# IST-DASLab/qutlass

Hardware: AMD Instinct MI355X
Metric: TFLOP/s & %FP4-MFMA-peak, MXFP4 GEMM 4096x4096x4096, 1 MI355X (higher is better)
Workload: dtype fp4 (e2m1 x e2m1, e8m0 block scales, fp32 accumulate, bf16 out); 1 GPU; matmul_mxf4_bf16_tn 4096x4096x4096, gs=32 e8m0 scales (BASELINE.json configs[1]); parallelism=single GPU, clock_ramp=8000 untimed steps (~250 ms) before the 5 warmup steps

## Files before the change

### qutlass_amd/csrc/capi.hip

```cpp
#include <hip/hip_runtime.h>

#include <algorithm>
#include <atomic>
#include <chrono>
#include <cmath>
#include <cstdarg>
#include <cstdio>
#include <cstring>
#include <utility>

#include "../../include/qutlass_amd.h"
#include "gemm_mx.hip.h"
#include "gemm_mx_forms.hip.h"
#include "gemm_mx_deepp.hip.h"
#include "gemm_mx_deepp16.hip.h"
#if QAMD_BENCH
#include "lab/gemm_mx_duo.hip.h"
#include "lab/gemm_mx_deepp_lab.hip.h"
#endif
#include "gemm_mx_skinny.hip.h"
#include "gemm_mx_ks.hip.h"
#include "gemm_mx_os.hip.h"
#include "gemm_mx_os_w4a8.hip.h"
#include "gemm_mx_fusedq.hip.h"
// ... 90 lines not shown
#else
constexpr bool opt_hw_fp4() { return true; }
constexpr int opt_gemm_variant() { return 0; }
constexpr int opt_nvf4_variant() { return 0; }
constexpr int opt_splitk_wg() { return 0; }
constexpr int opt_splitk_min_kt() { return 32; }
constexpr int opt_transpose_nc() { return 0; }
constexpr int opt_pp_shift() { return 2; }
constexpr int opt_pp_flags() { return 1; }
constexpr int opt_quant_wg_per_cu() { return 0; }
constexpr int opt_splitk_force() { return 0; }
constexpr int opt_deepp_grid() { return 0; }
constexpr int opt_bwd_variant() { return 0; }
constexpr int opt_moe_sort_one_launch_max() { return 0; }
constexpr uint32_t* opt_dbg() { return nullptr; }
#endif

inline int64_t cdiv(int64_t a, int64_t b) { return (a + b - 1) / b; }

#if QAMD_DEF(1)
int chip_cus() {
  static std::atomic<int> cache[64];
  int dev = 0;
  if (hipGetDevice(&dev) != hipSuccess || dev < 0 || dev >= 64) return 256;
  int v = cache[dev].load(std::memory_order_relaxed);
  if (v <= 0) {
    int n = 0;
    if (hipDeviceGetAttribute(&n, hipDeviceAttributeMultiprocessorCount, dev) != hipSuccess || n <= 0) n = 256;
    cache[dev].store(n, std::memory_order_relaxed);
    v = n;
  }
  return v;
}
#else
int chip_cus();
#endif


template <class C, int PP>
int launch_gemm(GemmParams p, hipStream_t s) {
  p.tiles_m = (int)cdiv(p.M, C::BM);
  p.tiles_n = (int)cdiv(p.N, C::BN);
  p.raster_magic = raster_magic(p.tiles_n);
  if (PP != 7 && PP != 9) { p.ws = nullptr; p.splits = 1; p.ctr = nullptr; p.tag = 0; }
  hipLaunchKernelGGL((gemm_mx_kernel<C, PP>), dim3(p.tiles_m * p.tiles_n, p.splits), dim3(C::THREADS), 0, s, p);
  return check_launch("gemm_mx_kernel");
}

inline int deepp_grid(int tiles) {
  const int forced = opt_deepp_grid();
  if (forced > 0) return std::min(forced, tiles);
  const int cus = chip_cus();
  const int rounds = (tiles + cus - 1) / cus;
  const int g = ((tiles + rounds - 1) / rounds + 7) / 8 * 8;
  return std::min(std::min(g, cus), tiles);
}

template <class C, bool TRACE = false, int ST_AUX = 0, int LAB = 0, int ONEFORM = 0>
int launch_gemm_deepp(GemmParams p, hipStream_t s) {
  p.tiles_m = (int)cdiv(p.M, C::BM);
  p.tiles_n = (int)cdiv(p.N, C::BN);
  p.raster_magic = raster_magic(p.tiles_n);
  p.ws = nullptr; p.splits = 1; p.ctr = nullptr; p.tag = 0;
  const int grid = deepp_grid(p.tiles_m * p.tiles_n);
#if QAMD_BENCH
#ifdef QAMD_ROUTE_LABK
  if constexpr (!TRACE && LAB == 0) {
    hipLaunchKernelGGL((labk::gemm_mx_deepp_kernel<C, false, ST_AUX, 8>), dim3(grid), dim3(C::THREADS), 0, s, p);
    return check_launch("labk::gemm_mx_deepp_kernel");
  }
#endif
  if constexpr (TRACE || LAB != 0) {
    hipLaunchKernelGGL((labk::gemm_mx_deepp_kernel<C, TRACE, ST_AUX, LAB>), dim3(grid), dim3(C::THREADS), 0, s, p);
    return check_launch("labk::gemm_mx_deepp_kernel");
  }
#else
  static_assert(!TRACE && LAB == 0, "traces / ablations: lab build only");
#endif
  const int64_t kt = cdiv((int64_t)p.K * C::EBITS / 8, 128);
  const bool odd = (kt & 1) && kt >= 3, one = grid == p.tiles_m * p.tiles_n;
  if (odd && one) hipLaunchKernelGGL((gemm_mx_deepp_kernel<C, ST_AUX, true, true>), dim3(grid), dim3(C::THREADS), 0, s, p);
  else if (odd) hipLaunchKernelGGL((gemm_mx_deepp_kernel<C, ST_AUX, true, false>), dim3(grid), dim3(C::THREADS), 0, s, p);
  else if (one) {
    static_assert(ONEFORM == 0 || ONEFORM == 16 || ONEFORM == 32, "one-tile form");
    static_assert(ONEFORM == 0 || QAMD_BENCH, "forced one-tile forms: lab build only");
    if constexpr (ONEFORM == 16 || (ONEFORM == 0 && kDeeppOneTile16)) hipLaunchKernelGGL((gemm_mx_deepp16_kernel<C, ST_AUX>), dim3(grid), dim3(C::THREADS), 0, s, p);
    else hipLaunchKernelGGL((gemm_mx_deepp_kernel<C, ST_AUX, false, true>), dim3(grid), dim3(C::THREADS), 0, s, p);
  }
  else hipLaunchKernelGGL((gemm_mx_deepp_kernel<C, ST_AUX>), dim3(grid), dim3(C::THREADS), 0, s, p);
  return check_launch("gemm_mx_deepp_kernel");
}

#if QAMD_BENCH
template <class C, int ST_AUX = 17, int RET = 0, bool TRACE = false>
int launch_gemm_duo(GemmParams p, hipStream_t s) {
  p.tiles_m = (int)cdiv(p.M, C::BM);
  p.tiles_n = (int)cdiv(p.N, C::BN);
  p.raster_magic = raster_magic(p.tiles_n);
  p.ws = nullptr; p.splits = 1; p.ctr = nullptr; p.tag = 0;
  const int grid = deepp_grid(p.tiles_m * p.tiles_n);
  hipLaunchKernelGGL((gemm_mx_duo_kernel<C, ST_AUX, RET, TRACE>), dim3(grid), dim3(C::THREADS), 0, s, p);
  return check_launch("gemm_mx_duo_kernel");
}
#endif

template <int TM, int TN, int D = 8>
int launch_gemm_ks(GemmParams p, hipStream_t s) {
  using C = KsCfg<TM, TN, D>;
  p.tiles_m = (int)cdiv(p.M, TM);
  p.tiles_n = (int)cdiv(p.N, TN);
  p.ws = nullptr; p.splits = 1; p.ctr = nullptr; p.tag = 0;
  hipLaunchKernelGGL((gemm_mx_ks_kernel<C>), dim3(p.tiles_m * p.tiles_n), dim3(256), 0, s, p);
  return check_launch("gemm_mx_ks_kernel");
}

template <bool RM, int TN, int EBITS, int TM, int AFMT, bool GRP, class P>
void launch_os_by_stages(int64_t KT, dim3 grid, const P& p, hipStream_t s) {
  const dim3 block(256);
  constexpr int SMAX = TM == 32 ? 4 : 3;
  if (KT <= 4) hipLaunchKernelGGL((gemm_mx_os_kernel<OsCfg<1, TN, EBITS, TM, AFMT>, RM, false, GRP>), grid, block, 0, s, p);
  else if (KT <= 8) hipLaunchKernelGGL((gemm_mx_os_kernel<OsCfg<2, TN, EBITS, TM, AFMT>, RM, false, GRP>), grid, block, 0, s, p);
  else if (KT <= 12) hipLaunchKernelGGL((gemm_mx_os_kernel<OsCfg<3, TN, EBITS, TM, AFMT>, RM, false, GRP>), grid, block, 0, s, p);
  else if (KT <= 4 * SMAX) hipLaunchKernelGGL((gemm_mx_os_kernel<OsCfg<SMAX, TN, EBITS, TM, AFMT>, RM, false, GRP>), grid, block, 0, s, p);
  else hipLaunchKernelGGL((gemm_mx_os_kernel<OsCfg<SMAX, TN, EBITS, TM, AFMT>, RM, true, GRP>), grid, block, 0, s, p);
}
template <bool RM = false, int TN = 32, int EBITS = 4, int TM = 32, int AFMT = 0>
int launch_gemm_os(GemmParams p, hipStream_t s) {
  p.tiles_m = (int)cdiv(p.M, TM);
  p.tiles_n = (int)cdiv(p.N, TN);
  p.ws = nullptr; p.splits = 1; p.ctr = nullptr; p.tag = 0;
  launch_os_by_stages<RM, TN, EBITS, TM, AFMT, false>(cdiv((int64_t)p.K * EBITS / 8, 128), dim3(p.tiles_m * p.tiles_n), p, s);
  return check_launch("gemm_mx_os_kernel");
}
template <int EBITS = 4, int AFMT = 0, bool RM = false, int TN = 16>
int launch_gemm_os16(GemmParams p, hipStream_t s) {
  p.tiles_m = (int)cdiv(p.M, 16);
  p.tiles_n = (int)cdiv(p.N, TN);
  p.ws = nullptr; p.splits = 1; p.ctr = nullptr; p.tag = 0;
  const int64_t KT = cdiv((int64_t)p.K * EBITS / 8, 128);
  const dim3 grid(p.tiles_m * p.tiles_n), block(256);
  constexpr int STAGE = Os16Cfg<1, EBITS, AFMT, TN>::STAGE;
  constexpr int SFIT = 160 * 1024 / (4 * STAGE), SMAX = SFIT >= 8 ? 8 : SFIT >= 4 ? 4 : SFIT;
  static_assert(SMAX >= 3, "LDS budget");
  if (KT <= 4) hipLaunchKernelGGL((gemm_mx_os16_kernel<Os16Cfg<1, EBITS, AFMT, TN>, false, RM>), grid, block, 0, s, p);
  else if (KT <= 8) hipLaunchKernelGGL((gemm_mx_os16_kernel<Os16Cfg<2, EBITS, AFMT, TN>, false, RM>), grid, block, 0, s, p);
  else if (KT <= 16 && SMAX >= 4) hipLaunchKernelGGL((gemm_mx_os16_kernel<Os16Cfg<(SMAX >= 4 ? 4 : SMAX), EBITS, AFMT, TN>, false, RM>), grid, block, 0, s, p);
  else if (KT <= 4 * SMAX) hipLaunchKernelGGL((gemm_mx_os16_kernel<Os16Cfg<SMAX, EBITS, AFMT, TN>, false, RM>), grid, block, 0, s, p);
  else hipLaunchKernelGGL((gemm_mx_os16_kernel<Os16Cfg<SMAX, EBITS, AFMT, TN>, true, RM>), grid, block, 0, s, p);
  return check_launch("gemm_mx_os16_kernel");
}
inline const MxFormRow* os16_form(int64_t N, int64_t cus) {
  for (const MxFormRow& f : MX_FORMS)
    if (f.family == MXF_DECODE && cdiv(N, f.tn) <= cus) return &f;
  return nullptr;
}
inline int os16_wide_plan(int ebits, int64_t N, int64_t K, int64_t cus) {
  const MxFormRow* f = os16_form(N, cus);
  const int tn = f ? f->tn : 0;
  const int64_t KT = cdiv(K * ebits / 8, 128);
  if (ebits == 4) {
    if (tn == 32) return (KT >= 12 && KT <= 32) ? f->variant : 0;
    if (tn == 48) return (KT >= 8 && KT <= 24) ? f->variant : 0;
    if (tn == 56) return (KT >= 8 && KT <= 16) ? f->variant : 0;
    if (tn == 64) return (KT >= 8 && KT <= 16) ? f->variant : 0;
    return 0;
  }
  if (tn == 32) return (KT >= 16 && KT <= 64) ? f->variant : 0;
  if (tn == 48) return (KT >= 16 && KT <= 32) ? f->variant : 0;
  return 0;
// ... 255 lines not shown
    return launch_gemm_os<RM, F.tn, EBITS, F.tm, AFMT>(p, s);
  } else {
    static_assert(F.family == MXF_DECODE && Os16Cfg<1, EBITS, AFMT, F.tn>::TM == F.tm && Os16Cfg<1, EBITS, AFMT, F.tn>::TN == F.tn, "the decode configuration is the row's");
    return launch_gemm_os16<EBITS, AFMT, RM, F.tn>(p, s);
  }
}
template <int I, int EBITS, int AFMT, bool RM>
inline bool try_mx_row(int v, const GemmParams& p, hipStream_t s, int& rc) {
  if constexpr (MX_FORMS[I].product && (MX_FORMS[I].ops & mx_op(EBITS, AFMT, RM)) != 0) {
    if (v == MX_FORMS[I].variant) { rc = launch_mx_row<I, EBITS, AFMT, RM>(p, s); return true; }
  }
  return false;
}
template <int EBITS, int AFMT, bool RM, int... I>
int launch_mx_form(int v, const GemmParams& p, hipStream_t s, const char* name, std::integer_sequence<int, I...>) {
  int rc = 0;
  if ((try_mx_row<I, EBITS, AFMT, RM>(v, p, s, rc) || ...)) return rc;
  if (AFMT == 1) return fail(QAMD_ERR_INVALID, "%s: gemm_variant %d has no e5m2-operand instantiation", name, v);
  return fail(QAMD_ERR_INVALID, "%s: unknown gemm_variant %d", name, v);
}

#if QAMD_BENCH
template <int EBITS>
int dispatch_lab_variant(int v, const GemmParams& p, hipStream_t s, const char* name) {
  constexpr bool SPLIT = EBITS == 8;
  switch (v) {
    case 273: return launch_gemm<GemmCfg<128, 128, 2, 2, EBITS, SPLIT, 128, 3>, 9>(p, s);
    case 272: return launch_gemm<GemmCfg<64, 128, 2, 2, EBITS, SPLIT, 128, 3>, 9>(p, s);
    case 270: return launch_gemm<GemmCfg<64, 64, 2, 2, EBITS, SPLIT, 128, 3>, 9>(p, s);
    case 224 + 1000: return launch_gemm<GemmCfg<128, 128, 2, 2, EBITS, SPLIT, 128, 2>, 9>(p, s);
    case 373: return launch_gemm<GemmCfg<128, 128, 2, 4, EBITS, SPLIT, 0, 3>, 9>(p, s);
    case 374: return launch_gemm<GemmCfg<128, 128, 4, 2, EBITS, SPLIT, 0, 3>, 9>(p, s);
    case 325: return launch_gemm<GemmCfg<256, 128, 2, 2, EBITS, SPLIT, 0, 3>, 9>(p, s);
    case 326: return launch_gemm<GemmCfg<128, 256, 2, 2, EBITS, SPLIT, 0, 3>, 9>(p, s);
    case 327: return launch_gemm<GemmCfg<256, 128, 2, 2, EBITS, SPLIT, 0, 2>, 9>(p, s);
    case 76: return launch_gemm<GemmCfg<128, 128, 2, 2, EBITS, SPLIT, 0, 4>, 9>(p, s);
    case 79: return launch_gemm<GemmCfg<64, 128, 2, 2, EBITS, SPLIT, 0, 4>, 9>(p, s);
    case 224: return launch_gemm<GemmCfg<128, 128, 2, 2, EBITS, SPLIT>, 3>(p, s);
    case 225: return launch_gemm<GemmCfg<256, 128, 4, 2, EBITS, SPLIT>, 3>(p, s);
    case 227: return launch_gemm<GemmCfg<128, 64, 2, 2, EBITS, SPLIT>, 3>(p, s);
    case 228: return launch_gemm<GemmCfg<64, 128, 2, 2, EBITS, SPLIT>, 3>(p, s);
    case 229: return launch_gemm<GemmCfg<64, 64, 2, 2, EBITS, SPLIT>, 3>(p, s);
    case 170: return launch_gemm<GemmCfg<64, 64, 2, 2, EBITS, SPLIT, 0, 3>, 7>(p, s);
    case 171: return launch_gemm<GemmCfg<128, 64, 2, 2, EBITS, SPLIT, 0, 3>, 7>(p, s);
    case 172: return launch_gemm<GemmCfg<64, 128, 2, 2, EBITS, SPLIT, 0, 3>, 7>(p, s);
    case 173: return launch_gemm<GemmCfg<128, 128, 2, 2, EBITS, SPLIT, 0, 3>, 7>(p, s);
    case 1: return launch_gemm<GemmCfg<256, 256, 2, 4, EBITS, SPLIT>, 1>(p, s);
    case 2: return launch_gemm<GemmCfg<128, 128, 2, 2, EBITS, SPLIT>, 0>(p, s);
    case 3: return launch_gemm<GemmCfg<256, 128, 4, 2, EBITS, SPLIT>, 0>(p, s);
    case 4: return launch_gemm<GemmCfg<128, 256, 2, 4, EBITS, SPLIT>, 0>(p, s);
    case 5: return launch_gemm<GemmCfg<256, 256, 2, 4, EBITS, SPLIT>, 0>(p, s);
    case 20: return launch_gemm<GemmCfg<256, 256, 2, 4, EBITS, SPLIT>, 3>(p, s);
    case 26: return launch_gemm<GemmCfg<128, 256, 2, 4, EBITS, SPLIT>, 3>(p, s);
    case 74: return launch_gemm<GemmCfg<64, 64, 2, 2, EBITS, SPLIT, 0, 4>, 7>(p, s);
    case 75: return launch_gemm<GemmCfg<64, 64, 2, 2, EBITS, SPLIT, 0, 6>, 7>(p, s);
    case 80: return launch_gemm<GemmCfg<64, 64, 2, 2, EBITS, SPLIT, 1, 3>, 7>(p, s);
    case 81: return launch_gemm<GemmCfg<64, 64, 2, 2, EBITS, SPLIT, 2, 3>, 7>(p, s);
    case 82: return launch_gemm<GemmCfg<64, 64, 2, 2, EBITS, SPLIT, 32, 3>, 7>(p, s);
    case 83: return launch_gemm<GemmCfg<64, 64, 2, 2, EBITS, SPLIT, 34, 3>, 7>(p, s);
    case 84: return launch_gemm<GemmCfg<64, 64, 2, 2, EBITS, SPLIT, 35, 3>, 7>(p, s);
    case 78: return launch_gemm<GemmCfg<64, 64, 2, 2, EBITS, SPLIT, 16, 3>, 7>(p, s);
  }
  if constexpr (EBITS == 8) {
    if (v == 89) return launch_gemm_deepp_sk<GemmCfg<256, 256, 2, 2, 8, true>>(p, s);
    if (v == 30) return launch_gemm<GemmCfg<256, 256, 2, 2, 8, true>, 4>(p, s);
  }
  if constexpr (EBITS == 4) {
    if (v == 89) return launch_gemm_deepp_sk<GemmCfg<256, 256, 2, 2, 4, false>>(p, s);
    if (v == 99) return launch_gemm_hetero<GemmCfg<256, 256, 2, 2, 4, false>, GemmCfg<128, 128, 2, 2, 4, false, 0, 3>, 17>(p, s);
    if (v == 563 || v == 564) {
      const bool deep = cdiv(p.K, 256) > 24;
      if (v == 563) return deep ? launch_gemm_ks<64, 32, 6>(p, s) : launch_gemm_ks<64, 32, 4>(p, s);
      return deep ? launch_gemm_ks<64, 64, 6>(p, s) : launch_gemm_ks<64, 64, 4>(p, s);
    }
    if (v == 565) return launch_gemm_ks<32, 32, 4>(p, s);
    if (v == 566) return launch_gemm_ks<32, 32, 8>(p, s);
    if (v == 567) return launch_gemm_ks<32, 32, 6>(p, s);
    if (v == 88) return launch_gemm_duo<GemmCfg<256, 256, 2, 4, 4, false>, 17, 0>(p, s);
    if (v == 87) return launch_gemm_duo<GemmCfg<256, 256, 2, 4, 4, false>, 17, 1>(p, s);
    if (v == 86) return launch_gemm_duo<GemmCfg<256, 256, 2, 4, 4, false>, 17, 0, true>(p, s);
    if (v == 298) return launch_gemm_hetero<GemmCfg<256, 256, 2, 2, 4, false>, GemmCfg<128, 128, 2, 2, 4, false, 128, 4>, 17>(p, s);
    if (v == 190) return launch_gemm_deepp<GemmCfg<256, 256, 2, 2, 4, false>, false, 17, 0, 32>(p, s);
    if (v == 191) return launch_gemm_deepp<GemmCfg<256, 256, 2, 2, 4, false>, false, 17, 0, 16>(p, s);
    if (v == 91) return launch_gemm_deepp<GemmCfg<256, 256, 2, 2, 4, false>, true, 17>(p, s);
    if (v == 92) return launch_gemm_deepp<GemmCfg<256, 256, 2, 2, 4, false>, false, 2>(p, s);
    if (v == 93) return launch_gemm_deepp<GemmCfg<256, 256, 2, 2, 4, false>, false, 16>(p, s);
    if (v == 94) return launch_gemm_deepp<GemmCfg<256, 256, 2, 2, 4, false>, false, 0>(p, s);
    if (v == 95) return launch_gemm_deepp<GemmCfg<256, 256, 2, 2, 4, false>, false, 19>(p, s);
    if (v == 96) return launch_gemm_deepp<GemmCfg<256, 256, 2, 2, 4, false>, false, 1>(p, s);
    if (v == 97) return launch_gemm_deepp<GemmCfg<256, 256, 2, 2, 4, false>, false, 17, 1>(p, s);
    if (v == 197) return launch_gemm_deepp<GemmCfg<256, 256, 2, 2, 4, false>, false, 17, 2>(p, s);
    if (v == 297) return launch_gemm_deepp<GemmCfg<256, 256, 2, 2, 4, false>, false, 17, 3>(p, s);
    if (v == 397) return launch_gemm_deepp<GemmCfg<256, 256, 2, 2, 4, false>, false, 17, 4>(p, s);
    switch (v) {
      case 6: return launch_gemm<GemmCfg<256, 256, 2, 4, 4, false>, 2>(p, s);
      case 7: return launch_gemm<GemmCfg<128, 128, 2, 2, 4, false>, 2>(p, s);
      case 8: return launch_gemm<GemmCfg<256, 128, 4, 2, 4, false>, 2>(p, s);
      case 9: return launch_gemm<GemmCfg<128, 256, 2, 4, 4, false>, 2>(p, s);
      case 30: return launch_gemm<GemmCfg<256, 256, 2, 2, 4, false>, 4>(p, s);
      case 31: return launch_gemm<GemmCfg<256, 256, 2, 2, 4, false, 8>, 4>(p, s);
      case 32: return launch_gemm<GemmCfg<256, 256, 2, 2, 4, false, 9>, 4>(p, s);
      case 33: return launch_gemm<GemmCfg<256, 256, 2, 2, 4, false, 10>, 4>(p, s);
      case 34: return launch_gemm<GemmCfg<256, 256, 2, 2, 4, false, 40>, 4>(p, s);
      case 40: return launch_gemm<GemmCfg<256, 256, 2, 2, 4, false>, 5>(p, s);
      case 41: return launch_gemm<GemmCfg<256, 256, 2, 2, 4, false, 8>, 5>(p, s);
      case 42: return launch_gemm<GemmCfg<256, 256, 2, 2, 4, false, 9>, 5>(p, s);
      case 43: return launch_gemm<GemmCfg<256, 256, 2, 2, 4, false, 10>, 5>(p, s);
      case 50: return launch_gemm<GemmCfg<256, 256, 2, 4, 4, false, 64>, 3>(p, s);
      case 51: return launch_gemm<GemmCfg<256, 256, 2, 2, 4, false, 64>, 4>(p, s);
      case 52: return launch_gemm<GemmCfg<256, 256, 2, 2, 4, false, 64>, 5>(p, s);
      case 53: return launch_gemm<GemmCfg<256, 256, 2, 2, 4, false, 72>, 5>(p, s);
      case 54: return launch_gemm<GemmCfg<256, 256, 2, 2, 4, false, 73>, 5>(p, s);
      case 55: return launch_gemm<GemmCfg<256, 256, 2, 2, 4, false, 74>, 5>(p, s);
      case 56: return launch_gemm<GemmCfg<256, 256, 2, 2, 4, false, 104>, 5>(p, s);
      case 35: return launch_gemm<GemmCfg<256, 256, 2, 2, 4, false, 16>, 4>(p, s);
      case 36: return launch_gemm<GemmCfg<256, 256, 2, 2, 4, false, 17>, 4>(p, s);
      case 21: return launch_gemm<GemmCfg<256, 256, 2, 4, 4, false, 8>, 3>(p, s);
      case 22: return launch_gemm<GemmCfg<256, 256, 2, 4, 4, false, 9>, 3>(p, s);
      case 23: return launch_gemm<GemmCfg<256, 256, 2, 4, 4, false, 10>, 3>(p, s);
    }
  }
  if constexpr (EBITS == 4 && !SPLIT) {
    const int rc = dispatch_ablation_mx4(v, p, s);
    if (rc >= 0) return rc;
  }
  return fail(QAMD_ERR_INVALID, "%s: unknown gemm_variant %d", name, v);
}
#endif

template <int EBITS, int AFMT, bool RM>
int dispatch_variant(int v, const GemmParams& p, hipStream_t s, const char* name) {
#if QAMD_BENCH
  if constexpr (AFMT == 0 && !RM) {
    if (p.pp_flags & 4096) {
      const MxFormRow* f = mx_form(v);
      if (f && f->family == MXF_RING) v += 100;
      else if (f && f->family == MXF_PIPELINED && f->depth == 2) v += 200;
    }
    if (!mx_form(v)) return dispatch_lab_variant<EBITS>(v, p, s, name);
  }
#endif
  return launch_mx_form<EBITS, AFMT, RM>(v, p, s, name, std::make_integer_sequence<int, MX_NFORMS>());
}

int launch_nn_fused_a5(const GemmParams& p, hipStream_t s, bool per_tile)
#if QAMD_DEF(4)
{
#if QAMD_BENCH
  if (per_tile) return launch_gemm<GemmCfg<256, 256, 2, 2, 8, true, 0, 2, 1>, 6>(p, s);
#endif
  (void)per_tile;
  return launch_gemm_deepp8<GemmCfg<256, 256, 2, 2, 8, true, 0, 2, 1>, true>(p, s);
}
#else
;
#endif

#if QAMD_TU != 0
#if QAMD_TU == 2
template int dispatch_variant<4, 0, false>(int, const GemmParams&, hipStream_t, const char*);
#else
extern template int dispatch_variant<4, 0, false>(int, const GemmParams&, hipStream_t, const char*);
#endif
#if QAMD_TU == 3
template int dispatch_variant<8, 0, false>(int, const GemmParams&, hipStream_t, const char*);
#if QAMD_BENCH
// ... 1638 lines not shown
```

### qutlass_amd/csrc/gemm_mx_deepp16.hip.h

```cpp
#pragma once
#include "gemm_mx_deepp.hip.h"

namespace qamd {

constexpr bool kDeeppOneTile16 = true;

constexpr int deepp16_row_done_at(int s) { return (s >= 7 && s <= 63 && (s - 7) % 8 == 0) ? (s - 7) / 8 : -1; }

template <class C, int ST_AUX = 0>
__device__ __forceinline__ void gemm_mx_deepp16(char* smem, const GemmParams& p, const int bid, const int G, const int ntiles) {
  static_assert(C::EBITS == 4 && C::BM == 256 && C::BN == 256 && C::WAVES_M == 2 && C::WAVES_N == 2 && C::NSTAGE == 2 && C::PPW == 2,
                "persistent deep schedule: fp4, 256x256 tiles, 4 waves of 128x128");
  constexpr int MT = 8, NT = 8;
  constexpr int STAGE = C::STAGE_BYTES, OFF_SCR = DeepPCfg<C>::OFF_SCR;
  GemmCtx<C> cx(smem, p);
  const int lane = cx.lane, wave = cx.wave, r16 = lane & 15, kq = lane >> 4;
  const int KT = cx.KT, KTe = (KT + 1) & ~1, CB = cx.CB, rowbytes = cx.rowbytes;
  const int tile = xcd_remap(bid, G);

  auto fence = [&]() __attribute__((always_inline)) { __builtin_amdgcn_sched_barrier(0); };
  struct Desc { __amdgpu_buffer_rsrc_t a, b, s; };
  int m0, n0;
  {
    int tm, tn;
    raster_decode(tile < ntiles ? tile : ntiles - 1, p.tiles_m, p.tiles_n, p.raster_magic, tm, tn);
    m0 = uniform(tm * C::BM);
    n0 = uniform(tn * C::BN);
  }
  Desc cur;
  {
    const bool valid = tile < ntiles;
    const uint32_t a_off = (uint32_t)m0 * rowbytes, b_off = (uint32_t)n0 * rowbytes;
    const uint32_t sa_off = (uint32_t)(m0 >> 7) * CB * 512, sb_off = (uint32_t)(n0 >> 7) * CB * 512;
    cur.a = make_rsrc(p.A + a_off, valid ? p.a_bytes - a_off : 0u);
    cur.b = make_rsrc(p.B + b_off, valid ? p.b_bytes - b_off : 0u);
    cur.s = cx.sIsB ? make_rsrc(p.SFB + sb_off, valid ? p.sfb_bytes - sb_off : 0u) : make_rsrc(p.SFA + sa_off, valid ? p.sfa_bytes - sa_off : 0u);
  }

  v4f acc[MT][NT];
  v4i fa[2][MT], fb[2][NT];
  v4i xq[2][4];
  const int sh = 8 * kq;

  const int sw = (r16 >> 1) & 7;
  int rdF[2];
#pragma unroll
  for (int h = 0; h < 2; ++h) rdF[h] = (cx.wave_m * C::WTM + r16) * C::ROWB + (((4 * h + kq) ^ sw) << 4);
  const int rdBd = cx.rdBd;
  const int rdSA = C::OFF_S + (cx.wave_m * C::SCT) * 512 + r16 * 16, rdSB = C::OFF_S + (C::PA + cx.wave_n * C::SCT) * 512 + r16 * 16;
  static_assert(C::SCT == 2 && C::WTM == 128 && C::WTN == 128, "a wave's rows are one 128-row scale tile; a stage is two column tiles");

  typedef __attribute__((address_space(3))) const v4i* lds_v4i_t;
  uint32_t rbA = 0, rbB = 0;
  auto read_base = [&](const int buf, const int h) __attribute__((always_inline)) {
    rbA = (uint32_t)(uintptr_t)(lds_ptr_t)(smem + buf * STAGE + rdF[h]);
    rbB = rbA + (uint32_t)rdBd;
    asm volatile("" : "+v"(rbA), "+v"(rbB));
  };
  auto read_frag = [&](const int h, const int i) __attribute__((always_inline)) {
    if (i < MT) fa[h][i] = *(lds_v4i_t)(uintptr_t)(rbA + (uint32_t)(i * 16 * C::ROWB));
    else fb[h][i - MT] = *(lds_v4i_t)(uintptr_t)(rbB + (uint32_t)((i - MT) * 16 * C::ROWB));
  };
  auto read_raw = [&](const int buf, const int h, const int k) __attribute__((always_inline)) {
    xq[h][k] = *(const v4i*)(smem + buf * STAGE + (k < 2 ? rdSA : rdSB) + h * 512 + (k & 1) * 256);
  };
  auto shift1 = [&](const int h, const int k) __attribute__((always_inline)) {
    xq[h][k >> 2][k & 3] = (int)((unsigned)xq[h][k >> 2][k & 3] >> sh);
  };
  auto mfma1 = [&](const int h, const int m, const int n, const bool zero_c) __attribute__((always_inline)) {
    const v4i a = fa[h][m], b = fb[h][n];
    const int sb1 = xq[h][2 + (n & 1)][n >> 1], sa1 = xq[h][m & 1][m >> 1];
    if (zero_c)
      asm volatile("v_mfma_scale_f32_16x16x128_f8f6f4 %0, %1, %2, 0, %3, %4 op_sel_hi:[0,0,0] cbsz:4 blgp:4" : "=a"(acc[m][n]) : "v"(b), "v"(a), "v"(sb1), "v"(sa1));
    else
      asm volatile("v_mfma_scale_f32_16x16x128_f8f6f4 %0, %1, %2, %0, %3, %4 op_sel_hi:[0,0,0] cbsz:4 blgp:4" : "+a"(acc[m][n]) : "v"(b), "v"(a), "v"(sb1), "v"(sa1));
  };

  int vb0 = 0, vb1 = 0, vbS = 0;
  auto dma_prep = [&](int kt, bool valid) __attribute__((always_inline)) {
    int lastmask = (kt == KT - 1) ? -1 : 0;
    int oobm = (valid && kt < KT) ? 0 : -1;
    int oobs = (valid && kt * C::SCT + cx.colS < CB) ? 0 : -1;
    asm volatile("" : "+v"(lastmask), "+v"(oobm), "+v"(oobs));
    vb0 = (((cx.voffT[0] & lastmask) | (cx.voffAB[0] & ~lastmask)) & ~oobm) | ((int)0x80000000 & oobm);
    vb1 = (((cx.voffT[1] & lastmask) | (cx.voffAB[1] & ~lastmask)) & ~oobm) | ((int)0x80000000 & oobm);
    vbS = (cx.voffS & ~oobs) | ((int)0x80000000 & oobs);
  };
  auto dma_item = [&](const Desc& d, int kt, const int buf, const int item) __attribute__((always_inline)) {
    char* st = smem + buf * STAGE;
    if (item < 16) {
      const int t = item & 7, q = wave * 8 + t;
      const int v = ((t & 1) ? vb1 : vb0) + q * cx.rstep;
      __builtin_amdgcn_raw_ptr_buffer_load_lds(item < 8 ? d.a : d.b, (lds_ptr_t)(st + (item < 8 ? 0 : C::OFF_B) + q * 1024), 16, v, kt * C::ROWB, 0, QAMD_DMA_AUX);
    } else {
      __builtin_amdgcn_raw_ptr_buffer_load_lds(d.s, (lds_ptr_t)(st + C::OFF_S + wave * 1024), 16, vbS, kt * C::SCT * 512, 0, 0);
    }
  };
  auto dma_stage = [&](const Desc& d, int kt, bool valid, const int buf) __attribute__((always_inline)) {
    dma_prep(kt, valid);
#pragma unroll
    for (int i = 0; i < 17; ++i) dma_item(d, kt, buf, i);
  };

  auto half = [&](const int h, const bool zero_c, auto extra) __attribute__((always_inline)) {
    int i = 0;
#pragma unroll
    for (int m = 0; m < MT; ++m)
#pragma unroll
      for (int n = 0; n < NT; ++n) {
        mfma1(h, m, n, zero_c);
        extra(i);
        fence();
        ++i;
      }
  };
  auto fill = [&](const int buf, const int hs, const int i) __attribute__((always_inline)) {
    if (i < 32 && (i & 1)) read_frag(hs, i >> 1);
    if (i >= 33 && i < 40 && (i & 1)) read_raw(buf, hs, (i - 33) >> 1);
    if (i >= 46 && i < 62) shift1(hs, i - 46);
  };

  auto stage = [&](auto bufc, auto firstc, int ktl, bool dvalid, auto dmac) __attribute__((always_inline)) {
    constexpr int BUF = decltype(bufc)::value;
    constexpr bool FIRST = decltype(firstc)::value;
    constexpr bool DMA = decltype(dmac)::value;
    read_base(BUF, 1);
    half(0, FIRST, [&](const int i) __attribute__((always_inline)) {
      fill(BUF, 1, i);
      if (DMA && i == 42) dma_prep(ktl, dvalid);
      if (i == 63) read_base(BUF ^ 1, 0);
    });
    asm volatile("s_waitcnt vmcnt(0) lgkmcnt(0)" ::: "memory");
    __builtin_amdgcn_s_barrier();
    fence();
    half(1, false, [&](const int i) __attribute__((always_inline)) {
      fill(BUF ^ 1, 0, i);
      if (DMA && !(i & 1) && i < 34) dma_item(cur, ktl, BUF, i >> 1);
    });
  };

  char* scr = smem + OFF_SCR + wave * DeepPCfg<C>::SCR_PER_WAVE;
  const int scrW = r16 * 512 + ((kq ^ (r16 & 7)) << 4);
  const int rrl = lane >> 3, ccl = lane & 7;
  const int scrR = rrl * 512 + (ccl >> 2) * 128 + ((((2 * ccl) & 7) ^ rrl) << 4);
  const float alpha = *p.alpha;
  __amdgpu_buffer_rsrc_t rD;
  int stLane, colLim;
  {
    const int64_t left = ((int64_t)(p.M - m0) * p.ldd - n0) * 2;
    rD = make_rsrc(p.D + ((int64_t)m0 * p.ldd + n0), (uint32_t)(left > 0x7fffffffll ? 0x7fffffffll : left));
    stLane = ((cx.wave_m * C::WTM + rrl) * p.ldd + cx.wave_n * C::WTN + 8 * ccl) * 2;
    colLim = p.N - n0 - cx.wave_n * C::WTN - 8 * ccl;
  }
  auto retire_write = [&](const int m) __attribute__((always_inline)) {
    asm volatile("s_nop 15" ::: "memory");
#pragma unroll
    for (int n = 0; n < NT; ++n) *(v4f*)(scr + (scrW ^ ((n & 1) << 6)) + (n >> 1) * 128) = acc[m][n];
  };
  v4f rb[2][2];
  auto retire_read = [&](const int rh) __attribute__((always_inline)) {
#pragma unroll
    for (int ch = 0; ch < 2; ++ch) {
      rb[ch][0] = *(const v4f*)(scr + scrR + rh * 4096 + ch * 256);
      rb[ch][1] = *(const v4f*)(scr + (scrR ^ 16) + rh * 4096 + ch * 256);
    }
  };
  auto retire_store = [&](const int m, const int pass) __attribute__((always_inline)) {
    const int rh = pass >> 1, ch = pass & 1;
    const v4f lo = rb[ch][0], hi = rb[ch][1];
    v4i o;
    o[0] = (int)pack_bf16x2(lo[0] * alpha, lo[1] * alpha);
    o[1] = (int)pack_bf16x2(lo[2] * alpha, lo[3] * alpha);
    o[2] = (int)pack_bf16x2(hi[0] * alpha, hi[1] * alpha);
    o[3] = (int)pack_bf16x2(hi[2] * alpha, hi[3] * alpha);
    int ldd2 = p.ldd * 2;
    asm volatile("" : "+s"(ldd2));
    __builtin_amdgcn_raw_buffer_store_b128(__builtin_bit_cast(v4u, o), rD, (64 * ch < colLim) ? stLane : (int)0x80000000, (16 * m + 8 * rh) * ldd2 + 128 * ch, ST_AUX);
  };

  auto final_stage = [&]() __attribute__((always_inline)) {
    read_base(1, 1);
    half(0, false, [&](const int i) __attribute__((always_inline)) { fill(1, 1, i); });
    asm volatile("s_waitcnt vmcnt(0) lgkmcnt(0)" ::: "memory");
    __builtin_amdgcn_s_barrier();
    fence();
    static_for<0, 75>([&](auto sc) __attribute__((always_inline)) {
      constexpr int s = decltype(sc)::value;
      if constexpr (s < 64) mfma1(1, s / 8, s % 8, false);
      constexpr int d1 = s - 1, d3 = s - 3, d5 = s - 5, d6 = s - 6, d7 = s - 7, d9 = s - 9, d10 = s - 10;
      if constexpr (deepp16_row_done_at(d5) >= 0) retire_store(deepp16_row_done_at(d5), 0);
      if constexpr (deepp16_row_done_at(d6) >= 0) retire_store(deepp16_row_done_at(d6), 1);
      if constexpr (deepp16_row_done_at(d9) >= 0) retire_store(deepp16_row_done_at(d9), 2);
      if constexpr (deepp16_row_done_at(d10) >= 0) retire_store(deepp16_row_done_at(d10), 3);
      if constexpr (deepp16_row_done_at(d1) >= 0) retire_write(deepp16_row_done_at(d1));
      if constexpr (deepp16_row_done_at(d3) >= 0) retire_read(0);
      if constexpr (deepp16_row_done_at(d7) >= 0) retire_read(1);
      fence();
    });
  };

  using I0 = std::integral_constant<int, 0>;
  using I1 = std::integral_constant<int, 1>;
  using BT = std::integral_constant<bool, true>;
  using BF = std::integral_constant<bool, false>;

  dma_stage(cur, 0, true, 0);
  dma_stage(cur, 1, true, 1);
  asm volatile("s_waitcnt vmcnt(17)" ::: "memory");
  __builtin_amdgcn_s_barrier();
  fence();
#pragma unroll
  for (int k = 0; k < 4; ++k) read_raw(0, 0, k);
  read_base(0, 0);
#pragma unroll
  for (int i = 0; i < MT + NT; ++i) read_frag(0, i);
#pragma unroll
  for (int k = 0; k < 16; ++k) shift1(0, k);
  fence();

  stage(I0{}, BT{}, 2, true, BT{});
  int kt = 1;
  for (; kt + 4 < KTe; kt += 2) {
    stage(I1{}, BF{}, kt + 2, true, BT{});
    stage(I0{}, BF{}, kt + 3, true, BT{});
  }
  if (kt + 2 < KTe) {
    stage(I1{}, BF{}, kt + 2, true, BT{});
    stage(I0{}, BF{}, 0, false, BF{});
  }
  final_stage();
  asm volatile("s_waitcnt vmcnt(0)" ::: "memory");
}

template <class C, int ST_AUX = 0>
__global__ __launch_bounds__(C::THREADS) void gemm_mx_deepp16_kernel(const GemmParams p) {
  __shared__ __attribute__((aligned(16))) char smem[DeepPCfg<C>::LDS_BYTES];
  asm volatile("" :: "s"(p.A), "s"(p.D), "s"(p.K), "s"(p.b_bytes), "s"((int)gridDim.x));
  gemm_mx_deepp16<C, ST_AUX>(smem, p, (int)blockIdx.x, (int)gridDim.x, p.tiles_m * p.tiles_n);
}

}
```

Baseline: 4357 TFLOP/s.

## Fuse LDS-DMA issue into MFMA asm and spread loads in deepp16 K-loop

Result: faster. 4491 TFLOP/s, median of 6 (+3.1%).

```diff
diff --git a/qutlass_amd/csrc/capi.hip b/qutlass_amd/csrc/capi.hip
--- a/qutlass_amd/csrc/capi.hip
+++ b/qutlass_amd/csrc/capi.hip
@@ -196,9 +196,10 @@
   if (odd && one) hipLaunchKernelGGL((gemm_mx_deepp_kernel<C, ST_AUX, true, true>), dim3(grid), dim3(C::THREADS), 0, s, p);
   else if (odd) hipLaunchKernelGGL((gemm_mx_deepp_kernel<C, ST_AUX, true, false>), dim3(grid), dim3(C::THREADS), 0, s, p);
   else if (one) {
-    static_assert(ONEFORM == 0 || ONEFORM == 16 || ONEFORM == 32, "one-tile form");
+    static_assert(ONEFORM == 0 || ONEFORM == 16 || ONEFORM == 32 || (ONEFORM >= 160 && ONEFORM < 168), "one-tile form");
     static_assert(ONEFORM == 0 || QAMD_BENCH, "forced one-tile forms: lab build only");
-    if constexpr (ONEFORM == 16 || (ONEFORM == 0 && kDeeppOneTile16)) hipLaunchKernelGGL((gemm_mx_deepp16_kernel<C, ST_AUX>), dim3(grid), dim3(C::THREADS), 0, s, p);
+    if constexpr (ONEFORM >= 160) hipLaunchKernelGGL((gemm_mx_deepp16_kernel<C, ST_AUX, ONEFORM - 160>), dim3(grid), dim3(C::THREADS), 0, s, p);
+    else if constexpr (ONEFORM == 16 || (ONEFORM == 0 && kDeeppOneTile16)) hipLaunchKernelGGL((gemm_mx_deepp16_kernel<C, ST_AUX>), dim3(grid), dim3(C::THREADS), 0, s, p);
     else hipLaunchKernelGGL((gemm_mx_deepp_kernel<C, ST_AUX, false, true>), dim3(grid), dim3(C::THREADS), 0, s, p);
   }
   else hipLaunchKernelGGL((gemm_mx_deepp_kernel<C, ST_AUX>), dim3(grid), dim3(C::THREADS), 0, s, p);
@@ -620,6 +621,12 @@
     if (v == 298) return launch_gemm_hetero<GemmCfg<256, 256, 2, 2, 4, false>, GemmCfg<128, 128, 2, 2, 4, false, 128, 4>, 17>(p, s);
     if (v == 190) return launch_gemm_deepp<GemmCfg<256, 256, 2, 2, 4, false>, false, 17, 0, 32>(p, s);
     if (v == 191) return launch_gemm_deepp<GemmCfg<256, 256, 2, 2, 4, false>, false, 17, 0, 16>(p, s);
+    if (v == 192) return launch_gemm_deepp<GemmCfg<256, 256, 2, 2, 4, false>, false, 17, 0, 160>(p, s);
+    if (v == 193) return launch_gemm_deepp<GemmCfg<256, 256, 2, 2, 4, false>, false, 17, 0, 160 + KL_SCALES>(p, s);
+    if (v == 194) return launch_gemm_deepp<GemmCfg<256, 256, 2, 2, 4, false>, false, 17, 0, 160 + KL_DMA>(p, s);
+    if (v == 195) return launch_gemm_deepp<GemmCfg<256, 256, 2, 2, 4, false>, false, 17, 0, 160 + (KL_SCALES | KL_DMA)>(p, s);
+    if (v == 196) return launch_gemm_deepp<GemmCfg<256, 256, 2, 2, 4, false>, false, 17, 0, 160 + (KL_SCALES | KL_DMA | KL_SPREAD)>(p, s);
+    if (v == 197) return launch_gemm_deepp<GemmCfg<256, 256, 2, 2, 4, false>, false, 17, 0, 160 + (KL_DMA | KL_SPREAD)>(p, s);
     if (v == 91) return launch_gemm_deepp<GemmCfg<256, 256, 2, 2, 4, false>, true, 17>(p, s);
     if (v == 92) return launch_gemm_deepp<GemmCfg<256, 256, 2, 2, 4, false>, false, 2>(p, s);
     if (v == 93) return launch_gemm_deepp<GemmCfg<256, 256, 2, 2, 4, false>, false, 16>(p, s);
diff --git a/qutlass_amd/csrc/gemm_mx_deepp16.hip.h b/qutlass_amd/csrc/gemm_mx_deepp16.hip.h
--- a/qutlass_amd/csrc/gemm_mx_deepp16.hip.h
+++ b/qutlass_amd/csrc/gemm_mx_deepp16.hip.h
@@ -7,10 +7,46 @@
 
 constexpr int deepp16_row_done_at(int s) { return (s >= 7 && s <= 63 && (s - 7) % 8 == 0) ? (s - 7) / 8 : -1; }
 
-template <class C, int ST_AUX = 0>
+enum { KL_SCALES = 1, KL_DMA = 2, KL_SPREAD = 4 };
+constexpr int kDeepp16KLoop = KL_DMA | KL_SPREAD;
+
+constexpr int deepp16_kblock(bool interleaved, int s, int kq) { return interleaved ? 4 * (kq >> 1) + 2 * (kq & 1) + s : 4 * s + kq; }
+constexpr bool deepp16_kblocks_once(bool interleaved) {
+  unsigned seen = 0;
+  for (int s = 0; s < 2; ++s)
+    for (int kq = 0; kq < 4; ++kq) {
+      const unsigned bit = 1u << deepp16_kblock(interleaved, s, kq);
+      if (seen & bit) return false;
+      seen |= bit;
+    }
+  return seen == 0xffu;
+}
+static_assert(deepp16_kblocks_once(false) && deepp16_kblocks_once(true), "every one of a stage's 8 K-blocks goes to exactly one (MFMA, lane group)");
+constexpr int deepp16_item_at(bool spread, int i) {
+  return spread ? (i == 0 ? 0 : (i % 4 == 2 ? (i + 2) / 4 : -1)) : ((i % 2 == 0 && i < 34) ? i / 2 : -1);
+}
+
+#if QAMD_DMA_AUX == 0
+#define QAMD_DMA_AUX_ASM ""
+#elif QAMD_DMA_AUX == 1
+#define QAMD_DMA_AUX_ASM " sc0"
+#elif QAMD_DMA_AUX == 2
+#define QAMD_DMA_AUX_ASM " nt"
+#elif QAMD_DMA_AUX == 16
+#define QAMD_DMA_AUX_ASM " sc1"
+#elif QAMD_DMA_AUX == 17
+#define QAMD_DMA_AUX_ASM " sc0 sc1"
+#else
+#error "QAMD_DMA_AUX: spell the cache-policy bits for the LDS-DMA statement of gemm_mx_deepp16"
+#endif
+#define QAMD_MFMA16(SRC_C, OP_SEL) "v_mfma_scale_f32_16x16x128_f8f6f4 %0, %1, %2, " SRC_C ", %3, %4 " OP_SEL "op_sel_hi:[0,0,0] cbsz:4 blgp:4"
+
+template <class C, int ST_AUX = 0, int KL = kDeepp16KLoop>
 __device__ __forceinline__ void gemm_mx_deepp16(char* smem, const GemmParams& p, const int bid, const int G, const int ntiles) {
   static_assert(C::EBITS == 4 && C::BM == 256 && C::BN == 256 && C::WAVES_M == 2 && C::WAVES_N == 2 && C::NSTAGE == 2 && C::PPW == 2,
                 "persistent deep schedule: fp4, 256x256 tiles, 4 waves of 128x128");
+  static_assert((KL & ~7) == 0 && (!(KL & KL_SPREAD) || (KL & KL_DMA)), "K-loop form");
+  constexpr bool IL = (KL & KL_SCALES) != 0, LEAN = (KL & KL_DMA) != 0, SPREAD = (KL & KL_SPREAD) != 0;
   constexpr int MT = 8, NT = 8;
   constexpr int STAGE = C::STAGE_BYTES, OFF_SCR = DeepPCfg<C>::OFF_SCR;
   GemmCtx<C> cx(smem, p);
@@ -36,19 +72,34 @@
     cur.b = make_rsrc(p.B + b_off, valid ? p.b_bytes - b_off : 0u);
     cur.s = cx.sIsB ? make_rsrc(p.SFB + sb_off, valid ? p.sfb_bytes - sb_off : 0u) : make_rsrc(p.SFA + sa_off, valid ? p.sfa_bytes - sa_off : 0u);
   }
+  v4u dwA, dwB, dwS;
+  if constexpr (LEAN) {
+    auto words = [&](const uint8_t* base, const uint32_t bytes) __attribute__((always_inline)) {
+      const uint64_t u = (uint64_t)(uintptr_t)base;
+      v4u d = {(uint32_t)u, (uint32_t)(u >> 32) & 0xffffu, bytes, 0x00020000u};
+      return d;
+    };
+    const uint32_t a_off = (uint32_t)m0 * rowbytes, b_off = (uint32_t)n0 * rowbytes;
+    const uint32_t sa_off = (uint32_t)(m0 >> 7) * CB * 512, sb_off = (uint32_t)(n0 >> 7) * CB * 512;
+    dwA = words(p.A + a_off, p.a_bytes - a_off);
+    dwB = words(p.B + b_off, p.b_bytes - b_off);
+    dwS = cx.sIsB ? words(p.SFB + sb_off, p.sfb_bytes - sb_off) : words(p.SFA + sa_off, p.sfa_bytes - sa_off);
+  }
 
   v4f acc[MT][NT];
   v4i fa[2][MT], fb[2][NT];
   v4i xq[2][4];
   const int sh = 8 * kq;
+  int xs[2][MT + NT];
 
   const int sw = (r16 >> 1) & 7;
   int rdF[2];
 #pragma unroll
-  for (int h = 0; h < 2; ++h) rdF[h] = (cx.wave_m * C::WTM + r16) * C::ROWB + (((4 * h + kq) ^ sw) << 4);
+  for (int h = 0; h < 2; ++h) rdF[h] = (cx.wave_m * C::WTM + r16) * C::ROWB + ((deepp16_kblock(IL, h, kq) ^ sw) << 4);
   const int rdBd = cx.rdBd;
   const int rdSA = C::OFF_S + (cx.wave_m * C::SCT) * 512 + r16 * 16, rdSB = C::OFF_S + (C::PA + cx.wave_n * C::SCT) * 512 + r16 * 16;
   static_assert(C::SCT == 2 && C::WTM == 128 && C::WTN == 128, "a wave's rows are one 128-row scale tile; a stage is two column tiles");
+  const int rdS2A = rdSA + (kq >> 1) * 512 + 2 * (kq & 1), rdS2B = rdSB + (kq >> 1) * 512 + 2 * (kq & 1);
 
   typedef __attribute__((address_space(3))) const v4i* lds_v4i_t;
   uint32_t rbA = 0, rbB = 0;
@@ -67,13 +118,30 @@
   auto shift1 = [&](const int h, const int k) __attribute__((always_inline)) {
     xq[h][k >> 2][k & 3] = (int)((unsigned)xq[h][k >> 2][k & 3] >> sh);
   };
-  auto mfma1 = [&](const int h, const int m, const int n, const bool zero_c) __attribute__((always_inline)) {
+  auto read_scale = [&](const int buf, const int k) __attribute__((always_inline)) {
+    const int t = k & 7;
+    xs[buf][k] = *(const uint16_t*)(smem + buf * STAGE + (k < MT ? rdS2A : rdS2B) + (t & 1) * 256 + (t >> 1) * 4);
+  };
+  auto mfma1 = [&](const int h, const int m, const int n, const bool zero_c, const int sbuf) __attribute__((always_inline)) {
     const v4i a = fa[h][m], b = fb[h][n];
-    const int sb1 = xq[h][2 + (n & 1)][n >> 1], sa1 = xq[h][m & 1][m >> 1];
+    const int sb1 = IL ? xs[sbuf][MT + n] : xq[h][2 + (n & 1)][n >> 1], sa1 = IL ? xs[sbuf][m] : xq[h][m & 1][m >> 1];
     if (zero_c)
-      asm volatile("v_mfma_scale_f32_16x16x128_f8f6f4 %0, %1, %2, 0, %3, %4 op_sel_hi:[0,0,0] cbsz:4 blgp:4" : "=a"(acc[m][n]) : "v"(b), "v"(a), "v"(sb1), "v"(sa1));
+      asm volatile(QAMD_MFMA16("0", "") : "=a"(acc[m][n]) : "v"(b), "v"(a), "v"(sb1), "v"(sa1));
+    else if (IL && h == 1)
+      asm volatile(QAMD_MFMA16("%0", "op_sel:[1,1,0] ") : "+a"(acc[m][n]) : "v"(b), "v"(a), "v"(sb1), "v"(sa1));
     else
-      asm volatile("v_mfma_scale_f32_16x16x128_f8f6f4 %0, %1, %2, %0, %3, %4 op_sel_hi:[0,0,0] cbsz:4 blgp:4" : "+a"(acc[m][n]) : "v"(b), "v"(a), "v"(sb1), "v"(sa1));
+      asm volatile(QAMD_MFMA16("%0", "") : "+a"(acc[m][n]) : "v"(b), "v"(a), "v"(sb1), "v"(sa1));
+  };
+  auto mfma1_dma = [&](const int h, const int m, const int n, const int sbuf, const v4u d, const uint32_t lds, const int voff, const int soff)
+                       __attribute__((always_inline)) {
+    const v4i a = fa[h][m], b = fb[h][n];
+    const int sb1 = IL ? xs[sbuf][MT + n] : xq[h][2 + (n & 1)][n >> 1], sa1 = IL ? xs[sbuf][m] : xq[h][m & 1][m >> 1];
+    if (IL && h == 1)
+      asm volatile("s_mov_b32 m0, %5\n\t" QAMD_MFMA16("%0", "op_sel:[1,1,0] ") "\n\tbuffer_load_dwordx4 %6, %7, %8 offen lds" QAMD_DMA_AUX_ASM
+                   : "+a"(acc[m][n]) : "v"(b), "v"(a), "v"(sb1), "v"(sa1), "s"(lds), "v"(voff), "s"(d), "s"(soff) : "memory");
+    else
+      asm volatile("s_mov_b32 m0, %5\n\t" QAMD_MFMA16("%0", "") "\n\tbuffer_load_dwordx4 %6, %7, %8 offen lds" QAMD_DMA_AUX_ASM
+                   : "+a"(acc[m][n]) : "v"(b), "v"(a), "v"(sb1), "v"(sa1), "s"(lds), "v"(voff), "s"(d), "s"(soff) : "memory");
   };
 
   int vb0 = 0, vb1 = 0, vbS = 0;
@@ -96,19 +164,48 @@
       __builtin_amdgcn_raw_ptr_buffer_load_lds(d.s, (lds_ptr_t)(st + C::OFF_S + wave * 1024), 16, vbS, kt * C::SCT * 512, 0, 0);
     }
   };
+  int vq[8], vqS = cx.voffS;
+  if constexpr (LEAN) {
+#pragma unroll
+    for (int t = 0; t < 8; ++t) {
+      vq[t] = cx.voffAB[t & 1] + (wave * 8 + t) * cx.rstep;
+      asm volatile("" : "+v"(vq[t]));
+    }
+    asm volatile("" : "+v"(vqS));
+  }
+  auto lean_slot = [&](const int i, const int m, const int n, int kt, const int buf) __attribute__((always_inline)) {
+    const int item = deepp16_item_at(SPREAD, i);
+    if (item < 0) return false;
+    char* st = smem + buf * STAGE;
+    if (item < 16) {
+      const int t = item & 7, q = wave * 8 + t;
+      mfma1_dma(1, m, n, buf, item < 8 ? dwA : dwB, (uint32_t)(uintptr_t)(lds_ptr_t)(st + (item < 8 ? 0 : C::OFF_B) + q * 1024), vq[t], kt * C::ROWB);
+    } else {
+      mfma1_dma(1, m, n, buf, dwS, (uint32_t)(uintptr_t)(lds_ptr_t)(st + C::OFF_S + wave * 1024), vqS, kt * C::SCT * 512);
+    }
+    return true;
+  };
   auto dma_stage = [&](const Desc& d, int kt, bool valid, const int buf) __attribute__((always_inline)) {
     dma_prep(kt, valid);
 #pragma unroll
     for (int i = 0; i < 17; ++i) dma_item(d, kt, buf, i);
   };
 
-  auto half = [&](const int h, const bool zero_c, auto extra) __attribute__((always_inline)) {
+  auto handoff_wait = [&]() __attribute__((always_inline)) {
+    if constexpr (KL != 0) {
+      fence();
+      __builtin_amdgcn_s_waitcnt(0x0070);
+    } else {
+      asm volatile("s_waitcnt vmcnt(0) lgkmcnt(0)" ::: "memory");
+    }
+  };
+  auto half = [&](const int h, const bool zero_c, const int sbuf, auto extra, auto with) __attribute__((always_inline)) {
     int i = 0;
 #pragma unroll
     for (int m = 0; m < MT; ++m)
 #pragma unroll
       for (int n = 0; n < NT; ++n) {
-        mfma1(h, m, n, zero_c);
+        if (!with(i, m, n)) mfma1(h, m, n, zero_c, sbuf);
         extra(i);
         fence();
         ++i;
@@ -116,26 +213,34 @@
   };
   auto fill = [&](const int buf, const int hs, const int i) __attribute__((always_inline)) {
     if (i < 32 && (i & 1)) read_frag(hs, i >> 1);
-    if (i >= 33 && i < 40 && (i & 1)) read_raw(buf, hs, (i - 33) >> 1);
-    if (i >= 46 && i < 62) shift1(hs, i - 46);
-  };
+    if constexpr (IL) {
+      if (hs == 0 && i >= 33 && (i & 1)) read_scale(buf, (((i - 33) >> 1) + NT) & 15);
+    } else {
+      if (i >= 33 && i < 40 && (i & 1)) read_raw(buf, hs, (i - 33) >> 1);
+      if (i >= 46 && i < 62) shift1(hs, i - 46);
+    }
+  };
+  auto alone = [&](const int, const int, const int) __attribute__((always_inline)) { return false; };
 
   auto stage = [&](auto bufc, auto firstc, int ktl, bool dvalid, auto dmac) __attribute__((always_inline)) {
     constexpr int BUF = decltype(bufc)::value;
     constexpr bool FIRST = decltype(firstc)::value;
-    constexpr bool DMA = decltype(dmac)::value;
+    constexpr int DMA = decltype(dmac)::value;
     read_base(BUF, 1);
-    half(0, FIRST, [&](const int i) __attribute__((always_inline)) {
+    half(0, FIRST, BUF, [&](const int i) __attribute__((always_inline)) {
       fill(BUF, 1, i);
-      if (DMA && i == 42) dma_prep(ktl, dvalid);
+      if (DMA == 1 && i == 42) dma_prep(ktl, dvalid);
       if (i == 63) read_base(BUF ^ 1, 0);
-    });
-    asm volatile("s_waitcnt vmcnt(0) lgkmcnt(0)" ::: "memory");
+    }, alone);
+    handoff_wait();
     __builtin_amdgcn_s_barrier();
     fence();
-    half(1, false, [&](const int i) __attribute__((always_inline)) {
+    half(1, false, BUF, [&](const int i) __attribute__((always_inline)) {
       fill(BUF ^ 1, 0, i);
-      if (DMA && !(i & 1) && i < 34) dma_item(cur, ktl, BUF, i >> 1);
+      if (DMA == 1 && !(i & 1) && i < 34) dma_item(cur, ktl, BUF, i >> 1);
+    }, [&](const int i, const int m, const int n) __attribute__((always_inline)) {
+      if constexpr (DMA == 2) return lean_slot(i, m, n, ktl, BUF);
+      else return false;
     });
   };
 
@@ -180,13 +285,13 @@
 
   auto final_stage = [&]() __attribute__((always_inline)) {
     read_base(1, 1);
-    half(0, false, [&](const int i) __attribute__((always_inline)) { fill(1, 1, i); });
-    asm volatile("s_waitcnt vmcnt(0) lgkmcnt(0)" ::: "memory");
+    half(0, false, 1, [&](const int i) __attribute__((always_inline)) { fill(1, 1, i); }, alone);
+    handoff_wait();
     __builtin_amdgcn_s_barrier();
     fence();
     static_for<0, 75>([&](auto sc) __attribute__((always_inline)) {
       constexpr int s = decltype(sc)::value;
-      if constexpr (s < 64) mfma1(1, s / 8, s % 8, false);
+      if constexpr (s < 64) mfma1(1, s / 8, s % 8, false, 1);
       constexpr int d1 = s - 1, d3 = s - 3, d5 = s - 5, d6 = s - 6, d7 = s - 7, d9 = s - 9, d10 = s - 10;
       if constexpr (deepp16_row_done_at(d5) >= 0) retire_store(deepp16_row_done_at(d5), 0);
       if constexpr (deepp16_row_done_at(d6) >= 0) retire_store(deepp16_row_done_at(d6), 1);
@@ -201,6 +306,7 @@
 
   using I0 = std::integral_constant<int, 0>;
   using I1 = std::integral_constant<int, 1>;
+  using I2 = std::integral_constant<int, 2>;
   using BT = std::integral_constant<bool, true>;
   using BF = std::integral_constant<bool, false>;
 
@@ -209,34 +315,47 @@
   asm volatile("s_waitcnt vmcnt(17)" ::: "memory");
   __builtin_amdgcn_s_barrier();
   fence();
-#pragma unroll
-  for (int k = 0; k < 4; ++k) read_raw(0, 0, k);
+  if constexpr (IL) {
+#pragma unroll
+    for (int k = 0; k < MT + NT; ++k) read_scale(0, k);
+  } else {
+#pragma unroll
+    for (int k = 0; k < 4; ++k) read_raw(0, 0, k);
+  }
   read_base(0, 0);
 #pragma unroll
   for (int i = 0; i < MT + NT; ++i) read_frag(0, i);
-#pragma unroll
-  for (int k = 0; k < 16; ++k) shift1(0, k);
+  if constexpr (!IL) {
+#pragma unroll
+    for (int k = 0; k < 16; ++k) shift1(0, k);
+  }
   fence();
 
-  stage(I0{}, BT{}, 2, true, BT{});
+  stage(I0{}, BT{}, 2, true, I1{});
   int kt = 1;
+  if constexpr (LEAN) {
+    for (; kt + 4 < KT; kt += 2) {
+      stage(I1{}, BF{}, kt + 2, true, I2{});
+      stage(I0{}, BF{}, kt + 3, true, I2{});
+    }
+  }
   for (; kt + 4 < KTe; kt += 2) {
-    stage(I1{}, BF{}, kt + 2, true, BT{});
-    stage(I0{}, BF{}, kt + 3, true, BT{});
+    stage(I1{}, BF{}, kt + 2, true, I1{});
+    stage(I0{}, BF{}, kt + 3, true, I1{});
   }
   if (kt + 2 < KTe) {
-    stage(I1{}, BF{}, kt + 2, true, BT{});
-    stage(I0{}, BF{}, 0, false, BF{});
+    stage(I1{}, BF{}, kt + 2, true, I1{});
+    stage(I0{}, BF{}, 0, false, I0{});
   }
   final_stage();
   asm volatile("s_waitcnt vmcnt(0)" ::: "memory");
 }
 
-template <class C, int ST_AUX = 0>
+template <class C, int ST_AUX = 0, int KL = kDeepp16KLoop>
 __global__ __launch_bounds__(C::THREADS) void gemm_mx_deepp16_kernel(const GemmParams p) {
   __shared__ __attribute__((aligned(16))) char smem[DeepPCfg<C>::LDS_BYTES];
   asm volatile("" :: "s"(p.A), "s"(p.D), "s"(p.K), "s"(p.b_bytes), "s"((int)gridDim.x));
-  gemm_mx_deepp16<C, ST_AUX>(smem, p, (int)blockIdx.x, (int)gridDim.x, p.tiles_m * p.tiles_n);
-}
-
-}
+  gemm_mx_deepp16<C, ST_AUX, KL>(smem, p, (int)blockIdx.x, (int)gridDim.x, p.tiles_m * p.tiles_n);
+}
+
+}
```
